# lliutianc/MPVAE-1

Measured on NVIDIA B200. Metric: probit-ELBO fwd+bwd label-samples/s, higher is better.
Workload: dtype f32

## Files before the change

mpvae-1_b200/csrc/probit_rows.cu:

```cuda
#include <stdlib.h>

#include "common.cuh"
#include "fused_rows.cuh"
#include "philox.cuh"
#include "probit_math.cuh"
#include "rows.h"
#include "small_rows.cuh"

namespace mpv {

namespace {

constexpr int kThreads = 256;
constexpr int kWarps = 8;
constexpr int kST = 2;

struct BlockCounts { int npos, nneg; };

struct RowChunk { float y, fe, fx, nr[kST]; bool obs; };

template <bool MASKED>
__device__ __forceinline__ void load_chunk(RowChunk& in, const RowArgs& a, const float* __restrict__ yrow,
                                           const float* __restrict__ ferow, const float* __restrict__ fxrow, int c, int lane,
                                           int b, int s0) {
    const int l = (c << 5) + lane;
    if (l < a.L) {
        in.obs = !MASKED || a.mask[(size_t)b * a.L + l] != 0;
        in.y = in.obs ? yrow[l] : 0.0f; in.fe = ferow[l]; in.fx = fxrow[l];
#pragma unroll
        for (int i = 0; i < kST; ++i)
            in.nr[i] = (s0 + i < a.S) ? a.nr[row_of(a, s0 + i, b) * a.ldn + l] : 0.0f;
    }
}

template <int NT = kThreads, bool MASKED = false>
__device__ __forceinline__ BlockCounts count_labels(const float* __restrict__ yrow, const uint8_t* __restrict__ mrow, int L,
                                                    int* s_tmp) {
    constexpr int kWarps = NT / 32;
    const int tid = threadIdx.x, lane = tid & 31, warp = tid >> 5;
    int cp = 0, cn = 0;
    for (int l = tid; l < L; l += NT) {
        if (MASKED && mrow[l] == 0) continue;
        const float v = yrow[l];
        cp += (v == 1.0f);
        cn += (v == 0.0f);
    }
    cp = warp_sum(cp);
    cn = warp_sum(cn);
    if (lane == 0) { s_tmp[warp] = cp; s_tmp[kWarps + warp] = cn; }
    __syncthreads();
    BlockCounts c{0, 0};
#pragma unroll
    for (int w = 0; w < kWarps; ++w) { c.npos += s_tmp[w]; c.nneg += s_tmp[kWarps + w]; }
    return c;
}

template <int NT = kThreads, bool MASKED = false>
__device__ __forceinline__ void row_tail(const RowArgs& a, int b) {
    constexpr int kWarps = NT / 32;
    __shared__ int s_cnt[2 * kWarps];
    __shared__ double s_kl[kWarps];
    __shared__ double s_fin[8];
    __shared__ int s_last;
    const int tid = threadIdx.x, lane = tid & 31, warp = tid >> 5;
    const int S = a.S, B = a.B;
    const BlockCounts cnt = count_labels<NT, MASKED>(a.y + (size_t)b * a.L, MASKED ? a.mask + (size_t)b * a.L : nullptr,
                                                     a.L, s_cnt);
    {
        double kp = 0.0;
        const size_t o = (size_t)b * a.D;
        for (int d = tid; d < a.D; d += NT)
            kp += (double)kl_cell(a.fe_mu[o + d], a.fe_logvar[o + d], a.fx_mu[o + d], a.fx_logvar[o + d]).term;
        kp = warp_sum(kp);
        if (lane == 0) s_kl[warp] = kp;
    }
    __syncthreads();
    if (warp == 0) {
        const float norm5 = 5.0f * ((float)cnt.npos * (float)cnt.nneg);
        double outv[5];
#pragma unroll
        for (int q = 0; q < 2; ++q) {
            const LogMeanExp lme =
                warp_log_mean_exp(S, lane, [&](int s) { return (float)a.lp[((size_t)b * S + s) * 2 + q]; });
            const float m = lme.m, fse = lme.fse;
            outv[q] = (double)lme.nll;
            double cs = 0.0;
            for (int s = lane; s < S; s += 32) {
                const size_t o = (size_t)b * S + s;
                a.wts[o * 2 + q] = expf((float)a.lp[o * 2 + q] - m) / fse;
                const float pos = a.stat[o * 4 + 2 * q], neg = a.stat[o * 4 + 2 * q + 1];
                float v = (pos * neg) / norm5;
                if (isnan(v) || isinf(v)) v = 0.0f;
                cs += (double)v;
            }
            outv[2 + q] = warp_sum(cs);
        }
        double kl = 0.0;
#pragma unroll
        for (int w = 0; w < kWarps; ++w) kl += s_kl[w];
        outv[4] = 0.5 * kl;
        if (lane == 0) {
#pragma unroll
            for (int q = 0; q < 5; ++q) a.rowout[(size_t)b * 8 + q] = outv[q];
            a.rowaux[(size_t)b * 2 + 0] = (float)cnt.npos;
            a.rowaux[(size_t)b * 2 + 1] = (float)cnt.nneg;
        }
    }
    __threadfence();
    __syncthreads();
    if (tid == 0) s_last = (atomicAdd(a.counter, 1u) == gridDim.x - 1);
    __syncthreads();
    if (!s_last) return;
    __threadfence();
    if (warp < 5) {
        double acc = 0.0;
        for (int r = lane; r < B; r += 32) acc += __ldcg(&a.rowout[(size_t)r * 8 + warp]);
        acc = warp_sum(acc);
        if (lane == 0) s_fin[warp] = acc;
    }
    __syncthreads();
    if (tid == 0) {
        const double dB = (double)B, dSB = (double)S * (double)B;
        const float nll = (float)(s_fin[0] / dB), nllx = (float)(s_fin[1] / dB);
        const float c = (float)(s_fin[2] / dSB), cx = (float)(s_fin[3] / dSB);
        const float kl = (float)(s_fin[4] / dB);
        const float total = MPV_ADD(MPV_ADD(MPV_MUL(MPV_ADD(nll, nllx), a.nll_coeff), MPV_MUL(MPV_ADD(c, cx), a.c_coeff)),
                                    MPV_MUL(kl, 1.1f));
        *a.scalars[0] = total; *a.scalars[1] = nll; *a.scalars[2] = nllx;
        *a.scalars[3] = c; *a.scalars[4] = cx; *a.scalars[5] = kl;
        *a.counter = 0u;
    }
}

template <bool MASKED>
__global__ void __launch_bounds__(kThreads, 4)
probit_row_finalize_kernel(const RowArgs a) {
    const int b = blockIdx.x;
    const int lane = threadIdx.x & 31, warp = threadIdx.x >> 5;
    for (int s = warp; s < a.S; s += kWarps) {
        const FusePart* __restrict__ pp = a.part + ((size_t)b * a.S + s) * a.part_tiles;
        double l0 = 0.0, l1 = 0.0;
        float q0 = 0.f, q1 = 0.f, q2 = 0.f, q3 = 0.f;
        for (int t = lane; t < a.part_tiles; t += 32) {
            const FusePart p = pp[t];
            l0 += p.lp_l; l1 += p.lp_x;
            q0 += p.pos_l; q1 += p.neg_l; q2 += p.pos_x; q3 += p.neg_x;
        }
        l0 = warp_sum(l0); l1 = warp_sum(l1);
        q0 = warp_sum(q0); q1 = warp_sum(q1); q2 = warp_sum(q2); q3 = warp_sum(q3);
        if (lane == 0) {
            const size_t o = (size_t)b * a.S + s;
            a.lp[o * 2 + 0] = l0; a.lp[o * 2 + 1] = l1;
            reinterpret_cast<float4*>(a.stat)[o] = make_float4(q0, q1, q2, q3);
        }
    }
    row_tail<kThreads, MASKED>(a, b);
}

constexpr int kChunk = 128;
constexpr int kLL = 4;

template <bool STABLE, int MINB, bool MASKED>
__global__ void __launch_bounds__(kThreads, MINB)
probit_row_fwd_tiled_kernel(const RowArgs a, FusePart* __restrict__ part, int nchunks) {
    const int b = blockIdx.x;
    const int lane = threadIdx.x & 31, warp = threadIdx.x >> 5;
    const int L = a.L, S = a.S;
    const size_t yoff = (size_t)b * L;
    const float fS = (float)S;
    for (int c = blockIdx.y * kWarps + warp; c < nchunks; c += gridDim.y * kWarps) {
        const int l0 = c * kChunk + kLL * lane;
        float y[kLL], fe[kLL], fx[kLL], accl[kLL], accx[kLL];
        bool obs[kLL];
#pragma unroll
        for (int j = 0; j < kLL; ++j) {
            y[j] = fe[j] = fx[j] = accl[j] = accx[j] = 0.f;
            if (l0 + j < L) { y[j] = a.y[yoff + l0 + j]; fe[j] = a.fe_out[yoff + l0 + j]; fx[j] = a.fx_out[yoff + l0 + j]; }
            if (MASKED) {
                obs[j] = l0 + j < L && a.mask[yoff + l0 + j] != 0;
                if (!obs[j]) y[j] = 0.f;
            }
        }
        const bool any = l0 < L;
        auto load = [&](int s) {
            float4 n = make_float4(0.f, 0.f, 0.f, 0.f);
            if (s < S && any) n = __ldcs(reinterpret_cast<const float4*>(a.nr + row_of(a, s, b) * a.ldn + l0));
            return n;
        };
        float4 n0 = load(0), n1 = load(1);
        for (int s0 = 0; s0 < S; s0 += kST) {
            const float4 m0 = load(s0 + 2), m1 = load(s0 + 3);
            float pl[kLL] = {0.f, 0.f, 0.f, 0.f}, px[kLL] = {0.f, 0.f, 0.f, 0.f};
            double lpl[kST], lpx[kST];
            float pn[kST][4];
#pragma unroll
            for (int i = 0; i < kST; ++i) {
                lpl[i] = lpx[i] = 0.0;
                pn[i][0] = pn[i][1] = pn[i][2] = pn[i][3] = 0.f;
                const int s = s0 + i;
                if (s >= S) continue;
                const float4 n4 = i == 0 ? n0 : n1;
                const float nv[kLL] = {n4.x, n4.y, n4.z, n4.w};
                float el[kLL], ex[kLL];
                float ll_l = 0.f, ll_x = 0.f;
#pragma unroll
                for (int j = 0; j < kLL; ++j) {
                    el[j] = ex[j] = 0.f;
                    if (l0 + j < L) {
                        const CellFwd cl = cell_forward<STABLE>(nv[j] + fe[j], y[j]);
                        const CellFwd cx = cell_forward<STABLE>(nv[j] + fx[j], y[j]);
                        if (!MASKED || obs[j]) {
                            lpl[i] += (double)cl.ll; lpx[i] += (double)cx.ll;
                            pn[i][0] += cl.epos; pn[i][1] += cl.eneg; pn[i][2] += cx.epos; pn[i][3] += cx.eneg;
                        }
                        pl[j] += cl.E; px[j] += cx.E;
                        el[j] = cl.E; ex[j] = cx.E;
                    }
                }
                (void)ll_l; (void)ll_x;
                if (a.E_l && any) {
                    const size_t o = row_of(a, s, b) * a.ldn + l0;
                    *reinterpret_cast<float4*>(a.E_l + o) = make_float4(el[0], el[1], el[2], el[3]);
                    *reinterpret_cast<float4*>(a.E_x + o) = make_float4(ex[0], ex[1], ex[2], ex[3]);
                }
            }
#pragma unroll
            for (int j = 0; j < kLL; ++j) { accl[j] += pl[j]; accx[j] += px[j]; }
#pragma unroll
            for (int i = 0; i < kST; ++i) {
                if (s0 + i >= S) continue;
                lpl[i] = warp_sum(lpl[i]); lpx[i] = warp_sum(lpx[i]);
#pragma unroll
                for (int q = 0; q < 4; ++q) pn[i][q] = warp_sum(pn[i][q]);
                if (lane == 0) {
                    FusePart p;
                    p.lp_l = lpl[i]; p.lp_x = lpx[i];
                    p.pos_l = pn[i][0]; p.neg_l = pn[i][1]; p.pos_x = pn[i][2]; p.neg_x = pn[i][3];
                    part[((size_t)b * S + s0 + i) * nchunks + c] = p;
                }
            }
            n0 = m0; n1 = m1;
        }
#pragma unroll
        for (int j = 0; j < kLL; ++j)
            if (l0 + j < L) {
                a.indiv_prob_label[yoff + l0 + j] = accl[j] / fS;
                a.indiv_prob[yoff + l0 + j] = accx[j] / fS;
            }
    }
}

struct RowCoeffs { float kb[2], cnb[2], a_kl; };

__device__ __forceinline__ RowCoeffs row_coeffs(const RowArgs& a, int b) {
    const float gt = a.g_scalars[0] ? *a.g_scalars[0] : 0.0f, g1 = a.g_scalars[1] ? *a.g_scalars[1] : 0.0f,
                g2 = a.g_scalars[2] ? *a.g_scalars[2] : 0.0f, g3 = a.g_scalars[3] ? *a.g_scalars[3] : 0.0f,
                g4 = a.g_scalars[4] ? *a.g_scalars[4] : 0.0f, g5 = a.g_scalars[5] ? *a.g_scalars[5] : 0.0f;
    const float a_nll[2] = {gt * a.nll_coeff + g1, gt * a.nll_coeff + g2};
    const float a_c[2] = {gt * a.c_coeff + g3, gt * a.c_coeff + g4};
    RowCoeffs rc;
    rc.a_kl = gt * 1.1f + g5;
    const float npos = a.rowaux[(size_t)b * 2], nneg = a.rowaux[(size_t)b * 2 + 1];
    const float norm5 = 5.0f * (npos * nneg);
    const float fS = (float)a.S, fB = (float)a.B;
#pragma unroll
    for (int q = 0; q < 2; ++q) {
        if (norm5 == 0.0f) {
            rc.kb[q] = a.sanitize ? 0.0f : __fdiv_rn(0.0f, norm5);
        } else {
            rc.kb[q] = (a_c[q] / (fS * fB)) / norm5;
        }
        rc.cnb[q] = -(a_nll[q] / fB);
    }
    return rc;
}

template <bool MASKED>
__global__ void __launch_bounds__(256)
gxs_bound_kernel(const RowArgs a, const unsigned int* __restrict__ gp_absmax, unsigned int* __restrict__ out_bits) {
    const int i = blockIdx.x * blockDim.x + threadIdx.x;
    unsigned int bits = 0u;
    if (i < a.B * a.S) {
        const int b = i / a.S;
        const RowCoeffs rc = row_coeffs(a, b);
        const float4 st = reinterpret_cast<const float4*>(a.stat)[i];
        const float2 w = reinterpret_cast<const float2*>(a.wts)[i];
        const float gp = gp_absmax ? (__uint_as_float(gp_absmax[0]) + __uint_as_float(gp_absmax[1])) / (float)a.S : 0.0f;
        float kl = fabsf(rc.kb[0]), kx = fabsf(rc.kb[1]);
        if (MASKED && a.rowaux[(size_t)b * 2] == 0.0f && a.rowaux[(size_t)b * 2 + 1] == 0.0f) kl = kx = 0.0f;
        const float bl = 5.0f * fabsf(rc.cnb[0] * w.x) + 17.0f * 5.0f * kl * fmaxf(st.x, st.y);
        const float bx = 5.0f * fabsf(rc.cnb[1] * w.y) + 17.0f * 5.0f * kx * fmaxf(st.z, st.w);
        bits = __float_as_uint(bl + bx + 0.4f * gp) & 0x7FFFFFFFu;
    }
#pragma unroll
    for (int o = 16; o > 0; o >>= 1) {
        const unsigned int t = __shfl_xor_sync(0xffffffffu, bits, o);
        bits = t > bits ? t : bits;
    }
    if ((threadIdx.x & 31) == 0 && bits != 0u) atomicMax(out_bits, bits);
}

template <bool STABLE, bool MASKED>
__global__ void __launch_bounds__(kThreads, 4)
probit_row_bwd_kernel(const RowArgs a) {
    extern __shared__ float s_gacc[];
    const int b = blockIdx.x;
    const int tid = threadIdx.x, lane = tid & 31, warp = tid >> 5;
    const int L = a.L, S = a.S, B = a.B;
    const int nwl = a.nwl, nws = kWarps / nwl;
    const int wl = warp % nwl, ws = warp / nwl;
    const int nchunks = (L + 31) >> 5;
    const float* __restrict__ yrow = a.y + (size_t)b * L;
    const float* __restrict__ ferow = a.fe_out + (size_t)b * L;
    const float* __restrict__ fxrow = a.fx_out + (size_t)b * L;

    for (int i = tid; i < nws * 2 * L; i += kThreads) s_gacc[i] = 0.0f;

    const RowCoeffs rc = row_coeffs(a, b);
    const float fS = (float)S, fB = (float)B;
    const float a_kl = rc.a_kl;
    const float* kb = rc.kb;
    const float* cnb = rc.cnb;
    const bool has_gp = a.g_indiv_prob != nullptr, has_gpl = a.g_indiv_prob_label != nullptr;
    const float gscale = a.gxs_planes ? scale_from_absmax_bits(*a.gxs_scale) : 1.0f;
    __syncthreads();

    unsigned int gmax = 0u;
    const int steps = (S + kST * nws - 1) / (kST * nws);
    for (int step = 0; step < steps; ++step) {
        const int s0 = (step * nws + ws) * kST;
        if (s0 >= S) continue;
        float cn[kST][2], cp[kST][2], cq[kST][2];
#pragma unroll
        for (int i = 0; i < kST; ++i) {
            const int s = min(s0 + i, S - 1);
            const size_t o = (size_t)b * S + s;
            const float4 st = reinterpret_cast<const float4*>(a.stat)[o];
            const float2 w = reinterpret_cast<const float2*>(a.wts)[o];
            cn[i][0] = cnb[0] * w.x;           cn[i][1] = cnb[1] * w.y;
            cp[i][0] = -5.0f * kb[0] * st.y;   cp[i][1] = -5.0f * kb[1] * st.w;
            cq[i][0] = 5.0f * kb[0] * st.x;    cq[i][1] = 5.0f * kb[1] * st.z;
        }
        float* __restrict__ gacc = s_gacc + (size_t)ws * 2 * L;
        RowChunk cur, nxt;
        int c = wl;
        if (c < nchunks) load_chunk<MASKED>(cur, a, yrow, ferow, fxrow, c, lane, b, s0);
        for (; c < nchunks; c += nwl) {
            if (c + nwl < nchunks) load_chunk<MASKED>(nxt, a, yrow, ferow, fxrow, c + nwl, lane, b, s0);
            const int l = (c << 5) + lane;
            if (l < L) {
                const float gpl = has_gpl ? a.g_indiv_prob_label[(size_t)b * L + l] / fS : 0.0f;
                const float gpx = has_gp ? a.g_indiv_prob[(size_t)b * L + l] / fS : 0.0f;
                float gl = 0.0f, gx = 0.0f;
#pragma unroll
                for (int i = 0; i < kST; ++i) {
                    if (s0 + i < S) {
                        float dl, dx;
                        if (!MASKED || cur.obs) {
                            dl = cell_backward<STABLE>(cur.nr[i] + cur.fe, cur.y, cn[i][0], cp[i][0], cq[i][0], gpl);
                            dx = cell_backward<STABLE>(cur.nr[i] + cur.fx, cur.y, cn[i][1], cp[i][1], cq[i][1], gpx);
                        } else {
                            dl = cell_backward<STABLE>(cur.nr[i] + cur.fe, 0.0f, 0.0f, 0.0f, 0.0f, gpl);
                            dx = cell_backward<STABLE>(cur.nr[i] + cur.fx, 0.0f, 0.0f, 0.0f, 0.0f, gpx);
                        }
                        gl += dl; gx += dx;
                        if (a.gxs_planes) {
                            const float g = (dl + dx) * gscale;
                            const __half hi = __float2half_rn(g);
                            __half* __restrict__ dst = a.gxs_planes + row_of(a, s0 + i, b) * a.gxs_pitch + l;
                            dst[0] = hi;
                            dst[a.gxs_plane_elems] = __float2half_rn(g - __half2float(hi));
                        } else if (a.gxs) {
                            const float g = dl + dx;
                            a.gxs[row_of(a, s0 + i, b) * a.ldn + l] = g;
                            const unsigned int gb = __float_as_uint(g) & 0x7FFFFFFFu;
                            gmax = gb > gmax ? gb : gmax;
                        }
                    }
                }
                gacc[l] += gl;
                gacc[L + l] += gx;
            }
            cur = nxt;
        }
    }
    if (a.gxs_planes) {
        const int pad = a.gxs_pitch - L;
        for (int i = tid; i < S * pad; i += kThreads) {
            __half* __restrict__ dst = a.gxs_planes + row_of(a, i / pad, b) * a.gxs_pitch + L + (i % pad);
            dst[0] = __float2half_rn(0.0f);
            dst[a.gxs_plane_elems] = __float2half_rn(0.0f);
        }
    }
    if (a.gxs_absmax && !a.gxs_planes) {
#pragma unroll
        for (int o = 16; o > 0; o >>= 1) {
            const unsigned int t = __shfl_xor_sync(0xffffffffu, gmax, o);
            gmax = t > gmax ? t : gmax;
        }
        if (lane == 0 && gmax != 0u) atomicMax(a.gxs_absmax, gmax);
    }
    __syncthreads();
    for (int l = tid; l < L; l += kThreads) {
        float sl = 0.0f, sx = 0.0f;
        for (int g = 0; g < nws; ++g) { sl += s_gacc[(size_t)g * 2 * L + l]; sx += s_gacc[(size_t)g * 2 * L + L + l]; }
        a.g_fe_out[(size_t)b * L + l] = sl;
        a.g_fx_out[(size_t)b * L + l] = sx;
    }
    const float kc = a_kl * 0.5f / fB;
    const size_t o = (size_t)b * a.D;
    for (int d = tid; d < a.D; d += kThreads) {
        const KlCell k = kl_cell(a.fe_mu[o + d], a.fe_logvar[o + d], a.fx_mu[o + d], a.fx_logvar[o + d]);
        a.g_fe_mu[o + d] = kc * k.d_fe_mu;
        a.g_fe_logvar[o + d] = kc * k.d_fe_lv;
        a.g_fx_mu[o + d] = kc * k.d_fx_mu;
        a.g_fx_logvar[o + d] = kc * k.d_fx_lv;
    }
}

template <bool MASKED>
__global__ void __launch_bounds__(kThreads, 4)
probit_row_bwd_saved_kernel(const RowArgs a) {
    extern __shared__ float s_coef[];
    const int b = blockIdx.x;
    const int tid = threadIdx.x, lane = tid & 31, warp = tid >> 5;
    const int L = a.L, S = a.S;
    const RowCoeffs rc = row_coeffs(a, b);
    for (int s = tid; s < S; s += kThreads) {
        const size_t o = (size_t)b * S + s;
        const float4 st = reinterpret_cast<const float4*>(a.stat)[o];
        const float2 w = reinterpret_cast<const float2*>(a.wts)[o];
        float* c = s_coef + s * 6;
        c[0] = rc.cnb[0] * w.x;           c[1] = rc.cnb[1] * w.y;
        c[2] = -5.0f * rc.kb[0] * st.y;   c[3] = -5.0f * rc.kb[1] * st.w;
        c[4] = 5.0f * rc.kb[0] * st.x;    c[5] = 5.0f * rc.kb[1] * st.z;
    }
    __syncthreads();
    const float fS = (float)S, fB = (float)a.B;
    const bool has_gp = a.g_indiv_prob != nullptr, has_gpl = a.g_indiv_prob_label != nullptr;
    const float gscale = a.gxs_planes ? scale_from_absmax_bits(*a.gxs_scale) : 1.0f;
    const int nchunks = a.gxs_planes ? a.gxs_pitch / 64 : (L + 63) / 64;
    const size_t yoff = (size_t)b * L;
    for (int c = blockIdx.y * kWarps + warp; c < nchunks; c += gridDim.y * kWarps) {
        const int l0 = c * 64 + 2 * lane;
        const bool in0 = l0 < L, in1 = l0 + 1 < L;
        float y0 = 0.f, y1 = 0.f, fe0 = 0.f, fe1 = 0.f, fx0 = 0.f, fx1 = 0.f, gpl0 = 0.f, gpl1 = 0.f, gpx0 = 0.f, gpx1 = 0.f;
        bool ob0 = true, ob1 = true;
        if (MASKED) { ob0 = in0 && a.mask[yoff + l0] != 0; ob1 = in1 && a.mask[yoff + l0 + 1] != 0; }
        if (in0) { if (ob0) y0 = a.y[yoff + l0]; fe0 = a.fe_out[yoff + l0]; fx0 = a.fx_out[yoff + l0]; }
        if (in1) { if (ob1) y1 = a.y[yoff + l0 + 1]; fe1 = a.fe_out[yoff + l0 + 1]; fx1 = a.fx_out[yoff + l0 + 1]; }
        if (has_gpl) { if (in0) gpl0 = a.g_indiv_prob_label[yoff + l0] / fS; if (in1) gpl1 = a.g_indiv_prob_label[yoff + l0 + 1] / fS; }
        if (has_gp) { if (in0) gpx0 = a.g_indiv_prob[yoff + l0] / fS; if (in1) gpx1 = a.g_indiv_prob[yoff + l0 + 1] / fS; }
        float gl0 = 0.f, gl1 = 0.f, gx0 = 0.f, gx1 = 0.f;
        const bool pair = l0 + 1 < a.ldn;
        struct Cell3 { float2 n, l, x; };
        auto load = [&](int s) {
            Cell3 v;
            v.n = v.l = v.x = make_float2(0.f, 0.f);
            if (s < S && in0) {
                const size_t o = row_of(a, s, b) * a.ldn + l0;
                if (pair) {
                    v.n = __ldcs(reinterpret_cast<const float2*>(a.nr + o));
                    v.l = __ldcs(reinterpret_cast<const float2*>(a.E_l + o));
                    v.x = __ldcs(reinterpret_cast<const float2*>(a.E_x + o));
                } else {
                    v.n.x = a.nr[o]; v.l.x = a.E_l[o]; v.x.x = a.E_x[o];
                }
            }
            return v;
        };
        Cell3 cur[2] = {load(0), load(1)};
        for (int s0 = 0; s0 < S; s0 += 2) {
            const Cell3 nxt[2] = {load(s0 + 2), load(s0 + 3)};
#pragma unroll
            for (int i = 0; i < 2; ++i) {
                const int s = s0 + i;
                if (s >= S) continue;
                const float* cf = s_coef + s * 6;
                const Cell3& v = cur[i];
                float d0 = 0.f, d1 = 0.f;
                if (in0) {
                    float dl, dx;
                    if (ob0) {
                        dl = cell_backward_saved(v.n.x + fe0, v.l.x, y0, cf[0], cf[2], cf[4], gpl0);
                        dx = cell_backward_saved(v.n.x + fx0, v.x.x, y0, cf[1], cf[3], cf[5], gpx0);
                    } else {
                        dl = cell_backward_saved(v.n.x + fe0, v.l.x, 0.0f, 0.0f, 0.0f, 0.0f, gpl0);
                        dx = cell_backward_saved(v.n.x + fx0, v.x.x, 0.0f, 0.0f, 0.0f, 0.0f, gpx0);
                    }
                    gl0 += dl; gx0 += dx; d0 = dl + dx;
                }
                if (in1) {
                    float dl, dx;
                    if (ob1) {
                        dl = cell_backward_saved(v.n.y + fe1, v.l.y, y1, cf[0], cf[2], cf[4], gpl1);
                        dx = cell_backward_saved(v.n.y + fx1, v.x.y, y1, cf[1], cf[3], cf[5], gpx1);
                    } else {
                        dl = cell_backward_saved(v.n.y + fe1, v.l.y, 0.0f, 0.0f, 0.0f, 0.0f, gpl1);
                        dx = cell_backward_saved(v.n.y + fx1, v.x.y, 0.0f, 0.0f, 0.0f, 0.0f, gpx1);
                    }
                    gl1 += dl; gx1 += dx; d1 = dl + dx;
                }
                if (a.gxs_planes) {
                    const float g0 = d0 * gscale, g1 = d1 * gscale;
                    const __half2 hi = __floats2half2_rn(g0, g1);
                    const float2 hf = __half22float2(hi);
                    const __half2 lo = __floats2half2_rn(g0 - hf.x, g1 - hf.y);
                    __half* __restrict__ dst = a.gxs_planes + row_of(a, s, b) * a.gxs_pitch + l0;
                    *reinterpret_cast<__half2*>(dst) = hi;
                    *reinterpret_cast<__half2*>(dst + a.gxs_plane_elems) = lo;
                } else if (a.gxs) {
                    const size_t o = row_of(a, s, b) * a.ldn + l0;
                    if (in0) a.gxs[o] = d0;
                    if (in1) a.gxs[o + 1] = d1;
                }
            }
            cur[0] = nxt[0]; cur[1] = nxt[1];
        }
        if (in0) { a.g_fe_out[yoff + l0] = gl0; a.g_fx_out[yoff + l0] = gx0; }
        if (in1) { a.g_fe_out[yoff + l0 + 1] = gl1; a.g_fx_out[yoff + l0 + 1] = gx1; }
    }
    if (blockIdx.y == 0) {
        const float kc = rc.a_kl * 0.5f / fB;
        const size_t o = (size_t)b * a.D;
        for (int d = tid; d < a.D; d += kThreads) {
            const KlCell k = kl_cell(a.fe_mu[o + d], a.fe_logvar[o + d], a.fx_mu[o + d], a.fx_logvar[o + d]);
            a.g_fe_mu[o + d] = kc * k.d_fe_mu;
            a.g_fe_logvar[o + d] = kc * k.d_fe_lv;
            a.g_fx_mu[o + d] = kc * k.d_fx_mu;
            a.g_fx_logvar[o + d] = kc * k.d_fx_lv;
        }
    }
}

template <bool STABLE, bool MASKED>
__global__ void __launch_bounds__(kSmallThreads)
probit_small_fwd_kernel(const SmallArgs p) {
    extern __shared__ __align__(16) unsigned char s_raw[];
    __shared__ __align__(8) unsigned long long s_bar;
    const RowArgs& a = p.a;
    const int b = blockIdx.x;
    const int tid = threadIdx.x, lane = tid & 31, warp = tid >> 5;
    const int L = a.L, S = a.S, Z = p.Z, B = a.B;
    const int npairs = (S + 1) >> 1;
    float* Rs = reinterpret_cast<float*>(s_raw);
    float* nz = Rs + (((size_t)L * Z + 3) & ~(size_t)3);
    float* ps = nz + (size_t)kSmallWarps * 2 * Z;
    const bool bulk = small_r_stage<kSmallThreads>(Rs, p.r, L, Z, &s_bar);
    const int nch = (L + 31) >> 5;
    float yv[4], fev[4], fxv[4];
    bool ov[4];
#pragma unroll
    for (int c = 0; c < 4; ++c) {
        const int l = (c << 5) + lane;
        yv[c] = fev[c] = fxv[c] = 0.f;
        if (c < nch && l < L) { yv[c] = a.y[(size_t)b * L + l]; fev[c] = a.fe_out[(size_t)b * L + l]; fxv[c] = a.fx_out[(size_t)b * L + l]; }
        if (MASKED) {
            ov[c] = c < nch && l < L && a.mask[(size_t)b * L + l] != 0;
            if (!ov[c]) yv[c] = 0.f;
        }
    }
    small_r_wait(bulk, &s_bar);
    __syncthreads();
    const uint2 off = philox_offset(p.off, p.off_dev);
    float* nzw = nz + (size_t)warp * 2 * Z;
    for (int pair = warp; pair < npairs; pair += kSmallWarps) {
        const int s0 = pair << 1;
        const bool two = s0 + 1 < S;
        small_noise_pair(nzw, p, s0, b, off, lane);
        __syncwarp();
        if (p.noise_out) {
            for (int i = 0; i < (two ? 2 : 1); ++i)
                for (int z = lane; z < Z; z += 32) p.noise_out[((size_t)(s0 + i) * B + b) * Z + z] = nzw[i * Z + z];
        }
        double lpl[2] = {0.0, 0.0}, lpx[2] = {0.0, 0.0};
        float pn[2][4] = {{0.f, 0.f, 0.f, 0.f}, {0.f, 0.f, 0.f, 0.f}};
#pragma unroll
        for (int c = 0; c < 4; ++c) {
            const int l = (c << 5) + lane;
            if (c >= nch || l >= L) continue;
            float acc0, acc1;
            small_nr_pair(Rs + (size_t)l * Z, nzw, Z, acc0, acc1);
            float pl = 0.f, px = 0.f;
#pragma unroll
            for (int i = 0; i < 2; ++i) {
                if (s0 + i >= S) continue;
                const float nr = i == 0 ? acc0 : acc1;
                const CellFwd cl = cell_forward<STABLE>(nr + fev[c], yv[c]);
                const CellFwd cx = cell_forward<STABLE>(nr + fxv[c], yv[c]);
                if (!MASKED || ov[c]) {
                    lpl[i] += (double)cl.ll; lpx[i] += (double)cx.ll;
                    pn[i][0] += cl.epos; pn[i][1] += cl.eneg; pn[i][2] += cx.epos; pn[i][3] += cx.eneg;
                }
                pl += cl.E; px += cx.E;
                if (p.nr_out) {
                    const size_t o = row_of(a, s0 + i, b) * a.ldn + l;
                    p.nr_out[o] = nr; a.E_l[o] = cl.E; a.E_x[o] = cx.E;
                }
            }
            ps[((size_t)pair * 2 + 0) * L + l] = pl;
            ps[((size_t)pair * 2 + 1) * L + l] = px;
        }
#pragma unroll
        for (int i = 0; i < 2; ++i) {
            if (s0 + i >= S) continue;
            lpl[i] = warp_sum(lpl[i]); lpx[i] = warp_sum(lpx[i]);
#pragma unroll
            for (int q = 0; q < 4; ++q) pn[i][q] = warp_sum(pn[i][q]);
            if (lane == 0) {
                const size_t o = (size_t)b * S + s0 + i;
                a.lp[o * 2 + 0] = lpl[i]; a.lp[o * 2 + 1] = lpx[i];
                reinterpret_cast<float4*>(a.stat)[o] = make_float4(pn[i][0], pn[i][1], pn[i][2], pn[i][3]);
            }
        }
        __syncwarp();
    }
    __syncthreads();
    const float fS = (float)S;
    for (int l = tid; l < L; l += kSmallThreads) {
        float sl = 0.f, sx = 0.f;
        for (int q = 0; q < npairs; ++q) { sl += ps[((size_t)q * 2 + 0) * L + l]; sx += ps[((size_t)q * 2 + 1) * L + l]; }
        a.indiv_prob_label[(size_t)b * L + l] = sl / fS;
        a.indiv_prob[(size_t)b * L + l] = sx / fS;
    }
    row_tail<kSmallThreads, MASKED>(a, b);
}

template <bool MASKED>
__global__ void __launch_bounds__(kThreads)
probit_small_bwd_kernel(const SmallArgs p) {
    extern __shared__ __align__(16) unsigned char s_raw[];
    const RowArgs& a = p.a;
    const int b = blockIdx.x;
    const int tid = threadIdx.x, lane = tid & 31, warp = tid >> 5;
    const int L = a.L, S = a.S, Z = p.Z, B = a.B;
    const int npairs = (S + 1) >> 1;
    float* coef = reinterpret_cast<float*>(s_raw);
    float* gxs = coef + (size_t)S * 6;
    float* nzs = gxs + (size_t)S * L;
    float* gsum = nzs + (size_t)S * Z;
    const RowCoeffs rc = row_coeffs(a, b);
    for (int s = tid; s < S; s += kThreads) {
        const size_t o = (size_t)b * S + s;
        const float4 st = reinterpret_cast<const float4*>(a.stat)[o];
        const float2 w = reinterpret_cast<const float2*>(a.wts)[o];
        float* c = coef + s * 6;
        c[0] = rc.cnb[0] * w.x;           c[1] = rc.cnb[1] * w.y;
        c[2] = -5.0f * rc.kb[0] * st.y;   c[3] = -5.0f * rc.kb[1] * st.w;
        c[4] = 5.0f * rc.kb[0] * st.x;    c[5] = 5.0f * rc.kb[1] * st.z;
    }
    const float* nsrc = p.noise_ext ? p.noise_ext : p.noise_out;
    for (int i = tid; i < S * Z; i += kThreads) nzs[i] = nsrc[((size_t)(i / Z) * B + b) * Z + (i % Z)];
    for (int i = tid; i < kWarps * 2 * L; i += kThreads) gsum[i] = 0.f;
    __syncthreads();
    const float fS = (float)S, fB = (float)B;
    const int nch = (L + 31) >> 5;
    for (int pair = warp; pair < npairs; pair += kWarps) {
#pragma unroll
        for (int c = 0; c < 4; ++c) {
            const int l = (c << 5) + lane;
            if (c >= nch || l >= L) continue;
            const bool ob = !MASKED || a.mask[(size_t)b * L + l] != 0;
            const float y = ob ? a.y[(size_t)b * L + l] : 0.f, fe = a.fe_out[(size_t)b * L + l], fx = a.fx_out[(size_t)b * L + l];
            const float gpl = a.g_indiv_prob_label ? a.g_indiv_prob_label[(size_t)b * L + l] / fS : 0.f;
            const float gpx = a.g_indiv_prob ? a.g_indiv_prob[(size_t)b * L + l] / fS : 0.f;
            float gl = 0.f, gx = 0.f;
            for (int i = 0; i < 2; ++i) {
                const int s = (pair << 1) + i;
                if (s >= S) break;
                const size_t o = row_of(a, s, b) * a.ldn + l;
                const float nr = a.nr[o];
                const float* cf = coef + s * 6;
                float dl, dx;
                if (ob) {
                    dl = cell_backward_saved(nr + fe, a.E_l[o], y, cf[0], cf[2], cf[4], gpl);
                    dx = cell_backward_saved(nr + fx, a.E_x[o], y, cf[1], cf[3], cf[5], gpx);
                } else {
                    dl = cell_backward_saved(nr + fe, a.E_l[o], 0.f, 0.f, 0.f, 0.f, gpl);
                    dx = cell_backward_saved(nr + fx, a.E_x[o], 0.f, 0.f, 0.f, 0.f, gpx);
                }
                gl += dl; gx += dx;
                gxs[(size_t)s * L + l] = dl + dx;
            }
            gsum[((size_t)warp * 2 + 0) * L + l] += gl;
            gsum[((size_t)warp * 2 + 1) * L + l] += gx;
        }
    }
    __syncthreads();
    for (int l = tid; l < L; l += kThreads) {
        float sl = 0.f, sx = 0.f;
        for (int w = 0; w < kWarps; ++w) { sl += gsum[((size_t)w * 2 + 0) * L + l]; sx += gsum[((size_t)w * 2 + 1) * L + l]; }
        a.g_fe_out[(size_t)b * L + l] = sl;
        a.g_fx_out[(size_t)b * L + l] = sx;
    }
    if (p.partial) {
        float* out = p.partial + (size_t)b * L * Z;
        for (int e = tid; e < L * Z; e += kThreads) {
            const int l = e / Z, z = e - l * Z;
            float acc = 0.f;
            for (int s = 0; s < S; ++s) acc = fmaf(gxs[(size_t)s * L + l], nzs[(size_t)s * Z + z], acc);
            out[e] = acc;
        }
    }
    const float kc = rc.a_kl * 0.5f / fB;
    const size_t o = (size_t)b * a.D;
    for (int d = tid; d < a.D; d += kThreads) {
        const KlCell k = kl_cell(a.fe_mu[o + d], a.fe_logvar[o + d], a.fx_mu[o + d], a.fx_logvar[o + d]);
        a.g_fe_mu[o + d] = kc * k.d_fe_mu;
        a.g_fe_logvar[o + d] = kc * k.d_fe_lv;
        a.g_fx_mu[o + d] = kc * k.d_fx_mu;
        a.g_fx_logvar[o + d] = kc * k.d_fx_lv;
    }
}

__global__ void __launch_bounds__(256)
small_gr_reduce_kernel(const float* __restrict__ partial, float* __restrict__ g_r, int B, int n) {
    const int e = blockIdx.x * blockDim.x + threadIdx.x;
    if (e >= n) return;
    float acc = 0.f;
    for (int b = 0; b < B; ++b) acc += partial[(size_t)b * n + e];
    g_r[e] = acc;
}

__global__ void log_normal_probe_kernel(const float* __restrict__ in, float* __restrict__ out, float* __restrict__ ref, size_t n) {
    for (size_t i = blockIdx.x * (size_t)blockDim.x + threadIdx.x; i < n; i += (size_t)gridDim.x * blockDim.x) {
        out[i] = MPV_LOG_NORMAL(in[i]);
        ref[i] = logf(in[i]);
    }
}

int pick_nwl(int L) {
    const int nchunks = (L + 31) / 32;
    int nwl = 1;
    while (nwl < nchunks && nwl < kWarps) nwl <<= 1;
    return nwl;
}

}

size_t row_smem_bytes(int L) {
    const int nwl = pick_nwl(L);
    return (size_t)(kWarps / nwl) * 2 * (size_t)L * sizeof(float);
}

int device_slot() {
    int d = 0;
    cudaGetDevice(&d);
    return (d >= 0 && d < kMaxDevices) ? d : 0;
}

static size_t small_fwd_smem(int S, int L, int Z) {
    return ((((size_t)L * Z + 3) & ~(size_t)3) + (size_t)kSmallWarps * 2 * Z + (size_t)((S + 1) / 2) * 2 * L) * sizeof(float);
}
static size_t small_bwd_smem(int S, int L, int Z) {
    return ((size_t)S * 6 + (size_t)S * L + (size_t)S * Z + (size_t)kWarps * 2 * L) * sizeof(float);
}
bool small_regime_fits(int S, int B, int L, int Z) {
    if (L > 128 || Z > 128 || L < 1 || Z < 1 || (long long)L * Z > 8192) return false;
    return small_fwd_smem(S, L, Z) <= 160 * 1024 && small_bwd_smem(S, L, Z) <= 160 * 1024;
}
size_t small_partial_bytes(int B, int L, int Z) { return (size_t)B * L * Z * sizeof(float); }

int launch_small_forward(RowArgs a, const SmallNoise& n, cudaStream_t stream) {
    const size_t smem = small_fwd_smem(a.S, a.L, n.Z);
    static bool configured[kMaxDevices] = {};
    const int dev = device_slot();
    if (!configured[dev]) {
        cudaError_t e = cudaFuncSetAttribute(probit_small_fwd_kernel<false, false>, cudaFuncAttributeMaxDynamicSharedMemorySize, 160 * 1024);
        if (e == cudaSuccess) e = cudaFuncSetAttribute(probit_small_fwd_kernel<true, false>, cudaFuncAttributeMaxDynamicSharedMemorySize, 160 * 1024);
        if (e == cudaSuccess) e = cudaFuncSetAttribute(probit_small_fwd_kernel<false, true>, cudaFuncAttributeMaxDynamicSharedMemorySize, 160 * 1024);
        if (e == cudaSuccess) e = cudaFuncSetAttribute(probit_small_fwd_kernel<true, true>, cudaFuncAttributeMaxDynamicSharedMemorySize, 160 * 1024);
        if (e == cudaSuccess) e = cudaFuncSetAttribute(probit_small_bwd_kernel<false>, cudaFuncAttributeMaxDynamicSharedMemorySize, 160 * 1024);
        if (e == cudaSuccess) e = cudaFuncSetAttribute(probit_small_bwd_kernel<true>, cudaFuncAttributeMaxDynamicSharedMemorySize, 160 * 1024);
        if (e != cudaSuccess) { set_error("cudaFuncSetAttribute(small): %s", cudaGetErrorString(e)); return 4; }
        configured[dev] = true;
    }
    const SmallArgs p = small_args(a, n);
    if (a.mask) {
        if (a.stable) probit_small_fwd_kernel<true, true><<<a.B, kSmallThreads, smem, stream>>>(p);
        else probit_small_fwd_kernel<false, true><<<a.B, kSmallThreads, smem, stream>>>(p);
    } else {
        if (a.stable) probit_small_fwd_kernel<true, false><<<a.B, kSmallThreads, smem, stream>>>(p);
        else probit_small_fwd_kernel<false, false><<<a.B, kSmallThreads, smem, stream>>>(p);
    }
    return check_launch("probit_small_fwd_kernel");
}

int launch_small_backward(RowArgs a, const SmallNoise& n, float* g_r, cudaStream_t stream) {
    const SmallArgs p = small_args(a, n);
    if (a.mask) probit_small_bwd_kernel<true><<<a.B, kThreads, small_bwd_smem(a.S, a.L, n.Z), stream>>>(p);
    else probit_small_bwd_kernel<false><<<a.B, kThreads, small_bwd_smem(a.S, a.L, n.Z), stream>>>(p);
    if (int rc = check_launch("probit_small_bwd_kernel")) return rc;
    if (g_r == nullptr) return 0;
    const int cnt = a.L * n.Z;
    small_gr_reduce_kernel<<<ceil_div(cnt, 256), 256, 0, stream>>>(n.partial, g_r, a.B, cnt);
    return check_launch("small_gr_reduce_kernel");
}

int launch_log_normal_probe(const float* in, float* out, float* ref, size_t n, cudaStream_t stream) {
    log_normal_probe_kernel<<<4 * kNumSMs, 256, 0, stream>>>(in, out, ref, n);
    return check_launch("log_normal_probe_kernel");
}

int row_chunks(int L) { return (L + kChunk - 1) / kChunk; }

int launch_row_forward(RowArgs a, cudaStream_t stream) {
    if (a.part == nullptr) { set_error("row forward: no scratch for the chunk partials"); return 1; }
    const int nchunks = row_chunks(a.L);
    int gy = ceil_div(2 * 2 * kNumSMs, a.B);
    if (gy > ceil_div(nchunks, kWarps)) gy = ceil_div(nchunks, kWarps);
    if (gy < 1) gy = 1;
    FusePart* part = const_cast<FusePart*>(a.part);
    const dim3 grid(a.B, gy);
    if (a.mask) {
        if (a.stable) probit_row_fwd_tiled_kernel<true, 2, true><<<grid, kThreads, 0, stream>>>(a, part, nchunks);
        else probit_row_fwd_tiled_kernel<false, 2, true><<<grid, kThreads, 0, stream>>>(a, part, nchunks);
    } else {
        if (a.stable) probit_row_fwd_tiled_kernel<true, 2, false><<<grid, kThreads, 0, stream>>>(a, part, nchunks);
        else probit_row_fwd_tiled_kernel<false, 2, false><<<grid, kThreads, 0, stream>>>(a, part, nchunks);
    }
    if (int rc = check_launch("probit_row_fwd_tiled_kernel")) return rc;
    a.part_tiles = nchunks;
    return launch_row_finalize(a, stream);
}

int launch_row_finalize(RowArgs a, cudaStream_t stream) {
    if (a.part == nullptr || a.part_tiles <= 0) { set_error("row finalize: no partials"); return 1; }
    if (a.mask) probit_row_finalize_kernel<true><<<a.B, kThreads, 0, stream>>>(a);
    else probit_row_finalize_kernel<false><<<a.B, kThreads, 0, stream>>>(a);
    return check_launch("probit_row_finalize_kernel");
}

int launch_gxs_bound(RowArgs a, const unsigned int* gp_absmax, unsigned int* out_bits, cudaStream_t stream) {
    if (a.mask) gxs_bound_kernel<true><<<ceil_div(a.B * a.S, 256), 256, 0, stream>>>(a, gp_absmax, out_bits);
    else gxs_bound_kernel<false><<<ceil_div(a.B * a.S, 256), 256, 0, stream>>>(a, gp_absmax, out_bits);
    return check_launch("gxs_bound_kernel");
}

int launch_row_backward(RowArgs a, cudaStream_t stream) {
    if (a.E_l != nullptr && a.E_x != nullptr && !a.stable) {
        const size_t smem = (size_t)a.S * 6 * sizeof(float);
        if (smem > 48 * 1024) { set_error("n_sample %d: per-sample coefficients exceed 48 KiB of shared memory", a.S); return 3; }
        const int nchunks = a.gxs_planes ? a.gxs_pitch / 64 : (a.L + 63) / 64;
        int gy = ceil_div(2 * 4 * kNumSMs, a.B);
        if (gy > ceil_div(nchunks, kWarps)) gy = ceil_div(nchunks, kWarps);
        if (gy < 1) gy = 1;
        if (a.mask) probit_row_bwd_saved_kernel<true><<<dim3(a.B, gy), kThreads, smem, stream>>>(a);
        else probit_row_bwd_saved_kernel<false><<<dim3(a.B, gy), kThreads, smem, stream>>>(a);
        return check_launch("probit_row_bwd_saved_kernel");
    }
    a.nwl = pick_nwl(a.L);
    const size_t smem = row_smem_bytes(a.L);
    if (smem > 200 * 1024) { set_error("label_dim %d needs %zu B of shared memory per row (limit 200 KiB)", a.L, smem); return 3; }
    static bool configured[kMaxDevices] = {};
    const int dev = device_slot();
    if (smem > 48 * 1024 && !configured[dev]) {
        cudaError_t e = cudaFuncSetAttribute(probit_row_bwd_kernel<false, false>, cudaFuncAttributeMaxDynamicSharedMemorySize, 200 * 1024);
        if (e == cudaSuccess) e = cudaFuncSetAttribute(probit_row_bwd_kernel<true, false>, cudaFuncAttributeMaxDynamicSharedMemorySize, 200 * 1024);
        if (e == cudaSuccess) e = cudaFuncSetAttribute(probit_row_bwd_kernel<false, true>, cudaFuncAttributeMaxDynamicSharedMemorySize, 200 * 1024);
        if (e == cudaSuccess) e = cudaFuncSetAttribute(probit_row_bwd_kernel<true, true>, cudaFuncAttributeMaxDynamicSharedMemorySize, 200 * 1024);
        if (e != cudaSuccess) { set_error("cudaFuncSetAttribute(bwd): %s", cudaGetErrorString(e)); return 4; }
        configured[dev] = true;
    }
    if (a.mask) {
        if (a.stable) probit_row_bwd_kernel<true, true><<<a.B, kThreads, smem, stream>>>(a);
        else probit_row_bwd_kernel<false, true><<<a.B, kThreads, smem, stream>>>(a);
    } else {
        if (a.stable) probit_row_bwd_kernel<true, false><<<a.B, kThreads, smem, stream>>>(a);
        else probit_row_bwd_kernel<false, false><<<a.B, kThreads, smem, stream>>>(a);
    }
    return check_launch("probit_row_bwd_kernel");
}

}
```

Measured before the change: 26.82 billion.

## Flatten row kernels into persistent tile grids and shrink finalize CTAs

```diff
diff --git a/mpvae-1_b200/csrc/probit_rows.cu b/mpvae-1_b200/csrc/probit_rows.cu
--- a/mpvae-1_b200/csrc/probit_rows.cu
+++ b/mpvae-1_b200/csrc/probit_rows.cu
@@ -55,25 +55,28 @@
     return c;
 }
 
-template <int NT = kThreads, bool MASKED = false>
+template <int NT = kThreads, bool MASKED = false, int KT = NT>
 __device__ __forceinline__ void row_tail(const RowArgs& a, int b) {
-    constexpr int kWarps = NT / 32;
+    constexpr int kWarps = NT / 32, kKlWarps = KT / 32;
+    static_assert(KT % NT == 0, "the KL order of a CTA of KT threads");
     __shared__ int s_cnt[2 * kWarps];
-    __shared__ double s_kl[kWarps];
+    __shared__ double s_kl[kKlWarps];
     __shared__ double s_fin[8];
     __shared__ int s_last;
     const int tid = threadIdx.x, lane = tid & 31, warp = tid >> 5;
     const int S = a.S, B = a.B;
     const BlockCounts cnt = count_labels<NT, MASKED>(a.y + (size_t)b * a.L, MASKED ? a.mask + (size_t)b * a.L : nullptr,
                                                      a.L, s_cnt);
-    {
+    auto kl_part = [&](int v, int first) {
         double kp = 0.0;
         const size_t o = (size_t)b * a.D;
-        for (int d = tid; d < a.D; d += NT)
+        for (int d = first; d < a.D; d += KT)
             kp += (double)kl_cell(a.fe_mu[o + d], a.fe_logvar[o + d], a.fx_mu[o + d], a.fx_logvar[o + d]).term;
         kp = warp_sum(kp);
-        if (lane == 0) s_kl[warp] = kp;
-    }
+        if (lane == 0) s_kl[v] = kp;
+    };
+    if constexpr (KT == NT) kl_part(warp, tid);
+    else for (int v = warp; v < kKlWarps; v += kWarps) kl_part(v, v * 32 + lane);
     __syncthreads();
     if (warp == 0) {
         const float norm5 = 5.0f * ((float)cnt.npos * (float)cnt.nneg);
@@ -97,7 +100,7 @@
         }
         double kl = 0.0;
 #pragma unroll
-        for (int w = 0; w < kWarps; ++w) kl += s_kl[w];
+        for (int w = 0; w < kKlWarps; ++w) kl += s_kl[w];
         outv[4] = 0.5 * kl;
         if (lane == 0) {
 #pragma unroll
@@ -112,12 +115,14 @@
     __syncthreads();
     if (!s_last) return;
     __threadfence();
-    if (warp < 5) {
+    auto batch_sum = [&](int q) {
         double acc = 0.0;
-        for (int r = lane; r < B; r += 32) acc += __ldcg(&a.rowout[(size_t)r * 8 + warp]);
+        for (int r = lane; r < B; r += 32) acc += __ldcg(&a.rowout[(size_t)r * 8 + q]);
         acc = warp_sum(acc);
-        if (lane == 0) s_fin[warp] = acc;
-    }
+        if (lane == 0) s_fin[q] = acc;
+    };
+    if constexpr (kWarps >= 5) { if (warp < 5) batch_sum(warp); }
+    else for (int q = warp; q < 5; q += kWarps) batch_sum(q);
     __syncthreads();
     if (tid == 0) {
         const double dB = (double)B, dSB = (double)S * (double)B;
@@ -132,12 +137,14 @@
     }
 }
 
+constexpr int kFinThreads = 128;
+
 template <bool MASKED>
-__global__ void __launch_bounds__(kThreads, 4)
+__global__ void __launch_bounds__(kFinThreads, 8)
 probit_row_finalize_kernel(const RowArgs a) {
     const int b = blockIdx.x;
     const int lane = threadIdx.x & 31, warp = threadIdx.x >> 5;
-    for (int s = warp; s < a.S; s += kWarps) {
+    for (int s = warp; s < a.S; s += kFinThreads / 32) {
         const FusePart* __restrict__ pp = a.part + ((size_t)b * a.S + s) * a.part_tiles;
         double l0 = 0.0, l1 = 0.0;
         float q0 = 0.f, q1 = 0.f, q2 = 0.f, q3 = 0.f;
@@ -154,7 +161,7 @@
             reinterpret_cast<float4*>(a.stat)[o] = make_float4(q0, q1, q2, q3);
         }
     }
-    row_tail<kThreads, MASKED>(a, b);
+    row_tail<kFinThreads, MASKED, kThreads>(a, b);
 }
 
 constexpr int kChunk = 128;
@@ -163,12 +170,13 @@
 template <bool STABLE, int MINB, bool MASKED>
 __global__ void __launch_bounds__(kThreads, MINB)
 probit_row_fwd_tiled_kernel(const RowArgs a, FusePart* __restrict__ part, int nchunks) {
-    const int b = blockIdx.x;
     const int lane = threadIdx.x & 31, warp = threadIdx.x >> 5;
     const int L = a.L, S = a.S;
-    const size_t yoff = (size_t)b * L;
     const float fS = (float)S;
-    for (int c = blockIdx.y * kWarps + warp; c < nchunks; c += gridDim.y * kWarps) {
+    const int tiles = a.B * nchunks;
+    for (int t = blockIdx.x * kWarps + warp; t < tiles; t += gridDim.x * kWarps) {
+        const int b = t / nchunks, c = t - b * nchunks;
+        const size_t yoff = (size_t)b * L;
         const int l0 = c * kChunk + kLL * lane;
         float y[kLL], fe[kLL], fx[kLL], accl[kLL], accx[kLL];
         bool obs[kLL];
@@ -418,30 +426,26 @@
     }
 }
 
+constexpr int kCoefWin = 32;
+
 template <bool MASKED>
 __global__ void __launch_bounds__(kThreads, 4)
 probit_row_bwd_saved_kernel(const RowArgs a) {
-    extern __shared__ float s_coef[];
-    const int b = blockIdx.x;
-    const int tid = threadIdx.x, lane = tid & 31, warp = tid >> 5;
+    __shared__ float s_coef[kWarps][kCoefWin * 6];
+    const int lane = threadIdx.x & 31, warp = threadIdx.x >> 5;
     const int L = a.L, S = a.S;
-    const RowCoeffs rc = row_coeffs(a, b);
-    for (int s = tid; s < S; s += kThreads) {
-        const size_t o = (size_t)b * S + s;
-        const float4 st = reinterpret_cast<const float4*>(a.stat)[o];
-        const float2 w = reinterpret_cast<const float2*>(a.wts)[o];
-        float* c = s_coef + s * 6;
-        c[0] = rc.cnb[0] * w.x;           c[1] = rc.cnb[1] * w.y;
-        c[2] = -5.0f * rc.kb[0] * st.y;   c[3] = -5.0f * rc.kb[1] * st.w;
-        c[4] = 5.0f * rc.kb[0] * st.x;    c[5] = 5.0f * rc.kb[1] * st.z;
-    }
-    __syncthreads();
+    float* __restrict__ wcoef = s_coef[warp];
     const float fS = (float)S, fB = (float)a.B;
     const bool has_gp = a.g_indiv_prob != nullptr, has_gpl = a.g_indiv_prob_label != nullptr;
     const float gscale = a.gxs_planes ? scale_from_absmax_bits(*a.gxs_scale) : 1.0f;
     const int nchunks = a.gxs_planes ? a.gxs_pitch / 64 : (L + 63) / 64;
-    const size_t yoff = (size_t)b * L;
-    for (int c = blockIdx.y * kWarps + warp; c < nchunks; c += gridDim.y * kWarps) {
+    const int tiles = a.B * nchunks, nw = gridDim.x * kWarps, gw = blockIdx.x * kWarps + warp;
+    const int per = tiles / nw, extra = tiles - per * nw;
+    const int t0 = gw * per + min(gw, extra), t1 = t0 + per + (gw < extra ? 1 : 0);
+    int built = -1;
+    for (int t = t0; t < t1; ++t) {
+        const int b = t / nchunks, c = t - b * nchunks;
+        const size_t yoff = (size_t)b * L;
         const int l0 = c * 64 + 2 * lane;
         const bool in0 = l0 < L, in1 = l0 + 1 < L;
         float y0 = 0.f, y1 = 0.f, fe0 = 0.f, fe1 = 0.f, fx0 = 0.f, fx1 = 0.f, gpl0 = 0.f, gpl1 = 0.f, gpx0 = 0.f, gpx1 = 0.f;
@@ -471,12 +475,28 @@
         };
         Cell3 cur[2] = {load(0), load(1)};
         for (int s0 = 0; s0 < S; s0 += 2) {
+            if ((s0 & (kCoefWin - 1)) == 0 && (b != built || S > kCoefWin)) {
+                __syncwarp();
+                const int s = s0 + lane;
+                if (s < S) {
+                    const RowCoeffs rc = row_coeffs(a, b);
+                    const size_t o = (size_t)b * S + s;
+                    const float4 st = reinterpret_cast<const float4*>(a.stat)[o];
+                    const float2 w = reinterpret_cast<const float2*>(a.wts)[o];
+                    float* cw = wcoef + lane * 6;
+                    cw[0] = rc.cnb[0] * w.x;           cw[1] = rc.cnb[1] * w.y;
+                    cw[2] = -5.0f * rc.kb[0] * st.y;   cw[3] = -5.0f * rc.kb[1] * st.w;
+                    cw[4] = 5.0f * rc.kb[0] * st.x;    cw[5] = 5.0f * rc.kb[1] * st.z;
+                }
+                __syncwarp();
+                built = b;
+            }
             const Cell3 nxt[2] = {load(s0 + 2), load(s0 + 3)};
 #pragma unroll
             for (int i = 0; i < 2; ++i) {
                 const int s = s0 + i;
                 if (s >= S) continue;
-                const float* cf = s_coef + s * 6;
+                const float* cf = wcoef + (s & (kCoefWin - 1)) * 6;
                 const Cell3& v = cur[i];
                 float d0 = 0.f, d1 = 0.f;
                 if (in0) {
@@ -519,16 +539,16 @@
         }
         if (in0) { a.g_fe_out[yoff + l0] = gl0; a.g_fx_out[yoff + l0] = gx0; }
         if (in1) { a.g_fe_out[yoff + l0 + 1] = gl1; a.g_fx_out[yoff + l0 + 1] = gx1; }
-    }
-    if (blockIdx.y == 0) {
-        const float kc = rc.a_kl * 0.5f / fB;
-        const size_t o = (size_t)b * a.D;
-        for (int d = tid; d < a.D; d += kThreads) {
-            const KlCell k = kl_cell(a.fe_mu[o + d], a.fe_logvar[o + d], a.fx_mu[o + d], a.fx_logvar[o + d]);
-            a.g_fe_mu[o + d] = kc * k.d_fe_mu;
-            a.g_fe_logvar[o + d] = kc * k.d_fe_lv;
-            a.g_fx_mu[o + d] = kc * k.d_fx_mu;
-            a.g_fx_logvar[o + d] = kc * k.d_fx_lv;
+        if (c == 0) {
+            const float kc = row_coeffs(a, b).a_kl * 0.5f / fB;
+            const size_t o = (size_t)b * a.D;
+            for (int d = lane; d < a.D; d += 32) {
+                const KlCell k = kl_cell(a.fe_mu[o + d], a.fe_logvar[o + d], a.fx_mu[o + d], a.fx_logvar[o + d]);
+                a.g_fe_mu[o + d] = kc * k.d_fe_mu;
+                a.g_fe_logvar[o + d] = kc * k.d_fe_lv;
+                a.g_fx_mu[o + d] = kc * k.d_fx_mu;
+                a.g_fx_logvar[o + d] = kc * k.d_fx_lv;
+            }
         }
     }
 }
@@ -804,30 +824,54 @@
 
 int row_chunks(int L) { return (L + kChunk - 1) / kChunk; }
 
+template <auto K>
+int tile_grid(int tiles) {
+    static int resident[kMaxDevices] = {};
+    const int dev = device_slot();
+    if (resident[dev] == 0) {
+        int d = 0, per_sm = 0, sms = 0;
+        cudaError_t e = cudaGetDevice(&d);
+        if (e == cudaSuccess) e = cudaOccupancyMaxActiveBlocksPerMultiprocessor(&per_sm, K, kThreads, 0);
+        if (e == cudaSuccess) e = cudaDeviceGetAttribute(&sms, cudaDevAttrMultiProcessorCount, d);
+        if (e != cudaSuccess || per_sm < 1) {
+            set_error("resident CTAs of a row kernel: %s", e != cudaSuccess ? cudaGetErrorString(e) : "none fit an SM");
+            return 0;
+        }
+        resident[dev] = per_sm * sms;
+    }
+    const int need = ceil_div(tiles, kWarps);
+    return need < 1 ? 1 : need < resident[dev] ? need : resident[dev];
+}
+
+template <auto K, typename... Args>
+int launch_tiles(int tiles, cudaStream_t stream, const Args&... args) {
+    const int grid = tile_grid<K>(tiles);
+    if (grid == 0) return 4;
+    K<<<grid, kThreads, 0, stream>>>(args...);
+    return 0;
+}
+
 int launch_row_forward(RowArgs a, cudaStream_t stream) {
     if (a.part == nullptr) { set_error("row forward: no scratch for the chunk partials"); return 1; }
-    const int nchunks = row_chunks(a.L);
-    int gy = ceil_div(2 * 2 * kNumSMs, a.B);
-    if (gy > ceil_div(nchunks, kWarps)) gy = ceil_div(nchunks, kWarps);
-    if (gy < 1) gy = 1;
+    const int nchunks = row_chunks(a.L), tiles = a.B * nchunks;
     FusePart* part = const_cast<FusePart*>(a.part);
-    const dim3 grid(a.B, gy);
+    int rc;
     if (a.mask) {
-        if (a.stable) probit_row_fwd_tiled_kernel<true, 2, true><<<grid, kThreads, 0, stream>>>(a, part, nchunks);
-        else probit_row_fwd_tiled_kernel<false, 2, true><<<grid, kThreads, 0, stream>>>(a, part, nchunks);
+        if (a.stable) rc = launch_tiles<probit_row_fwd_tiled_kernel<true, 2, true>>(tiles, stream, a, part, nchunks);
+        else rc = launch_tiles<probit_row_fwd_tiled_kernel<false, 2, true>>(tiles, stream, a, part, nchunks);
     } else {
-        if (a.stable) probit_row_fwd_tiled_kernel<true, 2, false><<<grid, kThreads, 0, stream>>>(a, part, nchunks);
-        else probit_row_fwd_tiled_kernel<false, 2, false><<<grid, kThreads, 0, stream>>>(a, part, nchunks);
-    }
-    if (int rc = check_launch("probit_row_fwd_tiled_kernel")) return rc;
+        if (a.stable) rc = launch_tiles<probit_row_fwd_tiled_kernel<true, 2, false>>(tiles, stream, a, part, nchunks);
+        else rc = launch_tiles<probit_row_fwd_tiled_kernel<false, 2, false>>(tiles, stream, a, part, nchunks);
+    }
+    if (rc || (rc = check_launch("probit_row_fwd_tiled_kernel"))) return rc;
     a.part_tiles = nchunks;
     return launch_row_finalize(a, stream);
 }
 
 int launch_row_finalize(RowArgs a, cudaStream_t stream) {
     if (a.part == nullptr || a.part_tiles <= 0) { set_error("row finalize: no partials"); return 1; }
-    if (a.mask) probit_row_finalize_kernel<true><<<a.B, kThreads, 0, stream>>>(a);
-    else probit_row_finalize_kernel<false><<<a.B, kThreads, 0, stream>>>(a);
+    if (a.mask) probit_row_finalize_kernel<true><<<a.B, kFinThreads, 0, stream>>>(a);
+    else probit_row_finalize_kernel<false><<<a.B, kFinThreads, 0, stream>>>(a);
     return check_launch("probit_row_finalize_kernel");
 }
 
@@ -839,14 +883,10 @@
 
 int launch_row_backward(RowArgs a, cudaStream_t stream) {
     if (a.E_l != nullptr && a.E_x != nullptr && !a.stable) {
-        const size_t smem = (size_t)a.S * 6 * sizeof(float);
-        if (smem > 48 * 1024) { set_error("n_sample %d: per-sample coefficients exceed 48 KiB of shared memory", a.S); return 3; }
         const int nchunks = a.gxs_planes ? a.gxs_pitch / 64 : (a.L + 63) / 64;
-        int gy = ceil_div(2 * 4 * kNumSMs, a.B);
-        if (gy > ceil_div(nchunks, kWarps)) gy = ceil_div(nchunks, kWarps);
-        if (gy < 1) gy = 1;
-        if (a.mask) probit_row_bwd_saved_kernel<true><<<dim3(a.B, gy), kThreads, smem, stream>>>(a);
-        else probit_row_bwd_saved_kernel<false><<<dim3(a.B, gy), kThreads, smem, stream>>>(a);
+        const int rc = a.mask ? launch_tiles<probit_row_bwd_saved_kernel<true>>(a.B * nchunks, stream, a)
+                              : launch_tiles<probit_row_bwd_saved_kernel<false>>(a.B * nchunks, stream, a);
+        if (rc) return rc;
         return check_launch("probit_row_bwd_saved_kernel");
     }
     a.nwl = pick_nwl(a.L);
```

Result: no change. 26.68 billion (median of 6 runs) (-0.5%).
